# akosiorek/sqair

Hardware: AMD Instinct MI355X
Metric: frames/sec (forward IWAE ELBO, 10-step 50x50 moving glyphs, K=5) (higher is better)
Workload: dtype f32; 1 GPU; cfg2: T=10 HxW=50x50 B=32/GPU K=5 N=4 cells VanillaRNN/GRU/GRU forward (elbo_iwae), HIP-graph replay=True; global_batch=32, seq_len=10, parallelism=dp1, graph_nodes=879

## Files before the change

### include/sqair_hip.h

```cpp
#ifndef SQAIR_HIP_H
#define SQAIR_HIP_H

#include <stddef.h>
#include <stdint.h>

#ifdef __cplusplus
extern "C" {
#endif

#define SQAIR_ABI_VERSION 2

typedef struct SqairConfig {
  int32_t img_h, img_w;
  int32_t glimpse_size;
  int32_t n_steps_per_image;
  int32_t n_what;
  int32_t n_hidden;
  int32_t k_particles;
  int32_t prop_prior_type;
  int32_t disc_prior_type;
  int32_t masked_glimpse;
  int32_t rec_where_prior;
  float prop_prior_step_bias;
  float step_success_prob;
// ... 543 lines not shown
} SqairWhereParamGradsTest;
int sqair_where_param_grads_test(SqairHandle* h, const SqairWhereParamGradsTest* t, void* stream);

typedef struct SqairGruGatesBwdTest {
  int32_t rows, accumulate_dh;
  const float* d_hn; int32_t dhn_ld;
  const float* z; int32_t z_ld;
  const float* r; int32_t r_ld;
  const float* hc; int32_t hc_ld;
  const float* hprev; int32_t h_ld;
  const float* d_rh; int32_t drh_ld;
  float* dpre1; int32_t dp_ld;
  float* d_h; int32_t dh_ld;
  float* dup_z; int32_t dupz_ld, dup_h_off;
  float* dup_r; int32_t dupr_ld;
} SqairGruGatesBwdTest;
int sqair_gru_gates_bwd_test(SqairHandle* h, const SqairGruGatesBwdTest* t, void* stream);

typedef struct SqairSlotCropTest {
  int32_t mode, slot, B, specialised;
  const float* img;
  const float* rec_prev; float* rec_new;
  const float* wb; int32_t wb_ld;
  const float* tp; int32_t tp_ld;
  const float* t2; int32_t t2_ld;
  const float* w3;
  const float* noise;
  const float* flat;
  const float* mask; int32_t mask_row_mul, mask_row_add;
  float* out; int32_t out_row_mul, out_row_add;
  float* tp_out; int32_t tp_out_ld;
} SqairSlotCropTest;
int sqair_slot_crop_test(SqairHandle* h, const SqairSlotCropTest* t, void* stream);

typedef struct SqairSlotTailTest {
  int32_t is_disc, slot, B, what_done;
  const float* hraw; int32_t h_ld;
  const float* enc; int32_t enc_ld;
  const float* rec_prev; float* rec_new;
  const float* noise;
  const float* s1p; int32_t s1p_ld;
  float* s1h_out; int32_t s1h_ld;
  const float* flat; const float* packed;
  const float* hid; int32_t hid_ld;
  const float* add; int32_t add_ld;
  float* out; int32_t out_ld;
} SqairSlotTailTest;
int sqair_slot_tail_test(SqairHandle* h, const SqairSlotTailTest* t, void* stream);

typedef struct SqairLinearWhatTest {
  int32_t mode, slot, B;
  const float* x; int32_t x_ld;
  const float* noise;
  const float* enc; int32_t enc_ld;
  const float* rec_prev; float* rec_new;
  const float* packed;
} SqairLinearWhatTest;
int sqair_linear_what_test(SqairHandle* h, const SqairLinearWhatTest* t, void* stream);

typedef struct SqairLogprobTest {
  int32_t B, T, t, t_global;
  const int32_t* t_row;
  const float* rec_p; const float* rec_d; const float* rec_prev;
  const float* pstats; int32_t ps_ld;
  const float* spre;
  const float* flat;
  float* qz; float* pz; float* disc_lp;
  const SqairOutputs* out;
} SqairLogprobTest;
int sqair_logprob_test(SqairHandle* h, const SqairLogprobTest* t, void* stream);

typedef struct SqairLogprobBwdTest {
  int32_t B, T, t_global0, ps_ld;
  const int32_t* t_row;
  const float* rec_p; const float* rec_d; const float* rec_m;
  const float* pstats; const float* spre;
  const float* g_lw; const float* g_dl;
  float* d_rec_p; float* d_rec_d; float* d_rec_m;
  float* d_pstats; float* d_spre;
  const float* flat; float* flat_grad;
} SqairLogprobBwdTest;
int sqair_logprob_bwd_test(SqairHandle* h, const SqairLogprobBwdTest* t, void* stream);

#define SQAIR_DENSE_ROUTES 23
int sqair_debug_dense_routes(int64_t* out, int n);

#ifdef __cplusplus
}
#endif
#endif
```

### sqair_amd/_capi.py

```python
from __future__ import annotations

import ctypes as C
import os

_HERE = os.path.dirname(os.path.abspath(__file__))
LIB_PATH = os.path.join(_HERE, "libsqair_hip.so")

OUTPUT_FIELDS = [
    "what", "what_loc", "what_scale", "where", "where_loc", "where_scale", "presence_prob", "presence",
    "presence_logit", "obj_id", "step_log_prob", "canvas", "glimpse", "disc_what_log_prob",
    "disc_where_log_prob", "disc_what_prior_log_prob", "disc_where_prior_log_prob", "disc_log_prob",
    "disc_prior_log_prob", "disc_prob", "prop_what_log_prob", "prop_where_log_prob",
    "prop_what_prior_log_prob", "prop_where_prior_log_prob", "prop_log_prob", "prop_prior_log_prob",
    "prop_prob", "discrete_log_prob", "num_prop_steps_per_sample", "num_disc_steps_per_sample",
    "num_steps_per_sample", "prop_pres", "disc_pres", "data_ll_per_sample", "kl_per_sample",
    "log_q_z_given_x_per_sample", "log_p_z_per_sample", "log_weights_per_timestep",
    "final_temporal_state", "final_prior_state", "final_last_used_id",
]
N_REFERENCE_OUTPUTS = 38


class SqairConfig(C.Structure):
    _fields_ = [
        ("img_h", C.c_int32), ("img_w", C.c_int32), ("glimpse_size", C.c_int32),
# ... 185 lines not shown


class SqairDenseContract(C.Structure):
    _fields_ = [("nseg", C.c_int32), ("seg", SqairDenseSeg * 4), ("w", C.c_void_p), ("b", C.c_void_p), ("add", C.c_void_p),
                ("add_ld", C.c_int32), ("add_n", C.c_int32), ("add_rdiv", C.c_int32), ("act_a", C.c_int32), ("act_b", C.c_int32),
                ("act_split", C.c_int32), ("scale", C.c_float), ("scale_ptr", C.c_void_p), ("out", C.c_void_p), ("out_ld", C.c_int32),
                ("M", C.c_int32), ("N", C.c_int32), ("scratch", C.c_void_p), ("scratch_bytes", C.c_int64)]


class SqairDxRange(C.Structure):
    _fields_ = [("n0", C.c_int32), ("n1", C.c_int32), ("dst", C.c_void_p), ("dst_ld", C.c_int32), ("dst2", C.c_void_p),
                ("dst2_ld", C.c_int32), ("add", C.c_void_p), ("add_ld", C.c_int32), ("saved", C.c_void_p), ("saved_ld", C.c_int32),
                ("act_a", C.c_int32), ("act_b", C.c_int32), ("act_split", C.c_int32)]


class SqairDxGru(C.Structure):
    _fields_ = [("mode", C.c_int32), ("g0", C.c_void_p), ("g0_ld", C.c_int32), ("g1", C.c_void_p), ("g1_ld", C.c_int32),
                ("hprev", C.c_void_p), ("h_ld", C.c_int32), ("dpre1", C.c_void_p), ("dp_ld", C.c_int32), ("d_h", C.c_void_p),
                ("dh_ld", C.c_int32), ("acc_dh", C.c_int32), ("dup", C.c_void_p), ("dup_ld", C.c_int32), ("dup_h_off", C.c_int32),
                ("nh", C.c_int32)]


class SqairDxTest(C.Structure):
    _fields_ = [("dpre", C.c_void_p), ("ld", C.c_int32), ("width", C.c_int32), ("M", C.c_int32), ("w", C.c_void_p),
                ("Kdim", C.c_int32), ("scale_ptr", C.c_void_p), ("nranges", C.c_int32), ("r", SqairDxRange * 3), ("gru", SqairDxGru),
                ("scratch", C.c_void_p), ("scratch_bytes", C.c_int64)]


def _fields(spec):
    return [(s.split()[1], C.c_void_p if s.split()[0] == "p" else C.c_int32) for s in spec]


class SqairSlotTailBwdTest(C.Structure):
    _fields_ = _fields(["i is_disc", "i slot", "i B", "i enc_pre", "p rec_prev", "p rec_new", "p d_rec_new", "p d_rec_prev", "p s1h",
                        "i s1h_ld", "p hraw", "i h_ld", "p enc", "i enc_ld", "p noise", "p flat", "p d_s1pre", "i ds_ld", "p d_s1pre2",
                        "i ds2_ld", "p d_raw_out", "i dr_ld", "p d_enc", "i de_ld", "p d_hraw", "i dh_ld"])


class SqairCropChainBwdTest(C.Structure):
    _fields_ = _fields(["i mode", "i slot", "i B", "i mask_dact", "p img", "p rec_prev", "p rec_new", "p d_rec_prev", "p d_rec_new", "p wb",
                        "i wb_ld", "p d_wb", "p mask", "i mask_row_mul", "i mask_row_add", "p d_mask", "p g_out", "i g_row_mul",
                        "i g_row_add", "p tp", "i tp_ld", "p d_tp", "i dtp_ld", "p noise", "p flat", "p w3", "p t2", "i t2_ld", "p d_t2",
                        "i dt2_ld"])


class SqairWhereParamGradsTest(C.Structure):
    _fields_ = _fields(["i T", "i B", "p d_tp", "i tp_ld", "p d_rec_p", "p rec_p", "p noise", "p flat_grad"])


class SqairGruGatesBwdTest(C.Structure):
    _fields_ = _fields(["i rows", "i accumulate_dh", "p d_hn", "i dhn_ld", "p z", "i z_ld", "p r", "i r_ld", "p hc", "i hc_ld", "p hprev",
                        "i h_ld", "p d_rh", "i drh_ld", "p dpre1", "i dp_ld", "p d_h", "i dh_ld", "p dup_z", "i dupz_ld", "i dup_h_off",
                        "p dup_r", "i dupr_ld"])


class SqairLogprobTest(C.Structure):
    _fields_ = _fields(["i B", "i T", "i t", "i t_global", "p t_row", "p rec_p", "p rec_d", "p rec_prev", "p pstats", "i ps_ld", "p spre",
                        "p flat", "p qz", "p pz", "p disc_lp", "p out"])


class SqairLogprobBwdTest(C.Structure):
    _fields_ = _fields(["i B", "i T", "i t_global0", "i ps_ld", "p t_row", "p rec_p", "p rec_d", "p rec_m", "p pstats", "p spre", "p g_lw",
                        "p g_dl", "p d_rec_p", "p d_rec_d", "p d_rec_m", "p d_pstats", "p d_spre", "p flat", "p flat_grad"])


class SqairSlotCropTest(C.Structure):
    _fields_ = _fields(["i mode", "i slot", "i B", "i specialised", "p img", "p rec_prev", "p rec_new", "p wb", "i wb_ld", "p tp", "i tp_ld",
                        "p t2", "i t2_ld", "p w3", "p noise", "p flat", "p mask", "i mask_row_mul", "i mask_row_add", "p out",
                        "i out_row_mul", "i out_row_add", "p tp_out", "i tp_out_ld"])


class SqairSlotTailTest(C.Structure):
    _fields_ = _fields(["i is_disc", "i slot", "i B", "i what_done", "p hraw", "i h_ld", "p enc", "i enc_ld", "p rec_prev", "p rec_new",
                        "p noise", "p s1p", "i s1p_ld", "p s1h_out", "i s1h_ld", "p flat", "p packed", "p hid", "i hid_ld", "p add",
                        "i add_ld", "p out", "i out_ld"])


class SqairLinearWhatTest(C.Structure):
    _fields_ = _fields(["i mode", "i slot", "i B", "p x", "i x_ld", "p noise", "p enc", "i enc_ld", "p rec_prev", "p rec_new", "p packed"])


DENSE_ROUTES = ("fwd_splitk", "fwd_t2", "fwd_rows", "fwd_mt", "fwd_lds", "fwd_big_2x2", "fwd_big_3x2", "fwd_big_3x3", "fwd_big_4x2",
                "dx_nch1", "dx_nch2", "dx_nch3", "dx_nch4", "dx_nch5", "dx_nch6", "dx_nch7", "dx_nch8", "dx_nch9", "dx_nch12", "dx_nch18",
                "dx_t2", "dx_gru1", "dx_gru2")


def dense_routes(library=None):
    v = (C.c_int64 * len(DENSE_ROUTES))()
    n = (library or lib()).sqair_debug_dense_routes(v, len(DENSE_ROUTES))
    assert n == len(DENSE_ROUTES), "the library counts {} dense routes, this binding names {}".format(n, len(DENSE_ROUTES))
    return dict(zip(DENSE_ROUTES, (int(x) for x in v)))


_PROTOS = {
    "sqair_abi_version": (C.c_int, []),
    "sqair_build_id": (C.c_char_p, []),
    "sqair_build_flags": (C.c_char_p, []),
    "sqair_create": (C.c_int, [C.POINTER(SqairConfig), C.POINTER(C.c_void_p)]),
    "sqair_destroy": (C.c_int, [C.c_void_p]),
    "sqair_last_error": (C.c_char_p, [C.c_void_p]),
    "sqair_param_count": (C.c_int64, [C.c_void_p]),
    "sqair_param_entries": (C.c_int, [C.c_void_p]),
    "sqair_param_entry": (C.c_int, [C.c_void_p, C.c_int, C.POINTER(C.c_char_p), C.POINTER(C.c_int64),
                                    C.POINTER(C.c_int64)]),
    "sqair_packed_bytes": (C.c_int64, [C.c_void_p]),
    "sqair_workspace_bytes": (C.c_int64, [C.c_void_p, C.c_int, C.c_int]),
    "sqair_noise_width": (C.c_int, [C.c_void_p]),
    "sqair_pack_params": (C.c_int, [C.c_void_p, C.c_void_p, C.c_void_p, C.c_void_p]),
    "sqair_forward": (C.c_int, [C.c_void_p, C.c_void_p, C.c_void_p, C.c_void_p, C.c_void_p, C.c_int, C.c_int,
                                C.c_int, C.POINTER(SqairOutputs), C.c_void_p, C.c_int64, C.c_void_p]),
    "sqair_train_workspace_bytes": (C.c_int64, [C.c_void_p, C.c_int, C.c_int]),
    "sqair_forward_train": (C.c_int, [C.c_void_p, C.c_void_p, C.c_void_p, C.c_void_p, C.c_void_p, C.c_int, C.c_int,
                                      C.c_int, C.POINTER(SqairOutputs), C.c_void_p, C.c_int64, C.c_void_p]),
    "sqair_graph_capture": (C.c_int, [C.c_void_p, C.c_void_p, C.c_void_p, C.c_void_p, C.c_void_p, C.c_int,
                                      C.c_int, C.c_int, C.POINTER(SqairOutputs), C.c_void_p, C.c_int64,
                                      C.c_void_p]),
    "sqair_graph_launch": (C.c_int, [C.c_void_p, C.c_void_p]),
    "sqair_graph_nodes": (C.c_int, [C.c_void_p]),
    "sqair_elbo": (C.c_int, [C.c_void_p, C.c_void_p, C.c_void_p, C.c_int, C.c_int, C.c_void_p, C.c_void_p,
                             C.c_void_p, C.c_void_p, C.c_void_p, C.POINTER(C.c_void_p), C.c_int, C.c_void_p,
                             C.c_void_p]),
    "sqair_st_crop": (C.c_int, [C.c_void_p, C.c_void_p, C.c_void_p, C.c_void_p, C.c_void_p, C.c_int, C.c_void_p]),
    "sqair_st_insert_loglik": (C.c_int, [C.c_void_p] * 8 + [C.c_int, C.c_void_p]),
    "sqair_linear_test": (C.c_int, [C.c_void_p, C.c_void_p, C.c_void_p, C.c_void_p, C.c_void_p, C.c_int, C.c_int,
                                    C.c_int, C.c_int, C.c_void_p, C.c_int64, C.c_void_p]),
    "sqair_gru_test": (C.c_int, [C.c_void_p, C.c_void_p, C.c_void_p, C.c_void_p, C.c_void_p, C.c_int, C.c_int,
                                 C.c_void_p, C.c_int64, C.c_void_p]),
    "sqair_set_workspace_clearing": (C.c_int, [C.c_void_p, C.c_int]),
    "sqair_clear_workspace": (C.c_int, [C.c_void_p, C.c_void_p, C.c_int64, C.c_int, C.c_int, C.c_int, C.c_void_p]),
    "sqair_set_option": (C.c_int, [C.c_void_p, C.c_char_p, C.c_int]),
    "sqair_chain_status": (C.c_int, [C.c_void_p, C.c_void_p, C.c_int, C.c_int, C.c_int, C.c_void_p]),
    "sqair_check_scales": (C.c_int, [C.c_void_p, C.c_void_p, C.c_int, C.c_int, C.c_int, C.c_void_p, C.c_void_p]),
    "sqair_check_finite": (C.c_int, [C.c_void_p, C.c_void_p, C.c_int64, C.c_char_p, C.c_void_p, C.c_void_p]),
    "sqair_timeline_available": (C.c_int, []),
    "sqair_timeline_begin": (C.c_int, [C.c_void_p, C.c_void_p, C.c_int64]),
    "sqair_timeline_count": (C.c_int, [C.c_void_p]),
    "sqair_timeline_end": (C.c_int, [C.c_void_p]),
    "sqair_timeline_record": (C.c_int, [C.c_void_p, C.c_int, C.POINTER(C.c_char_p), C.POINTER(C.c_int64), C.POINTER(C.c_int),
                                        C.POINTER(C.c_int)]),
    "sqair_lstm_test": (C.c_int, [C.c_void_p] * 6 + [C.c_int, C.c_int, C.c_void_p, C.c_int64, C.c_void_p]),
    "sqair_lstm_cell_bwd_test": (C.c_int, [C.c_void_p] * 7 + [C.c_int, C.c_void_p]),
    "sqair_compact_test_layout": (C.c_int, [C.c_void_p, C.POINTER(C.c_int32), C.c_int]),
    "sqair_compact_test": (C.c_int, [C.c_void_p] * 13 + [C.POINTER(SqairOutputs), C.c_int, C.c_int, C.c_void_p]),
    "sqair_compact_bwd_test": (C.c_int, [C.c_void_p] * 11 + [C.c_int, C.c_void_p]),
    "sqair_get_config":(C.c_int, [C.c_void_p, C.POINTER(SqairConfig)]),
    "sqair_st_crop_bwd": (C.c_int, [C.c_void_p] * 7 + [C.c_int, C.c_void_p]),
    "sqair_st_insert_loglik_bwd": (C.c_int, [C.c_void_p] * 11 + [C.c_int64, C.c_int, C.c_void_p]),
    "sqair_elbo_bwd": (C.c_int, [C.c_void_p, C.c_void_p, C.c_void_p, C.c_int, C.c_int, C.c_void_p, C.c_void_p,
                                 C.c_void_p]),
    "sqair_backward_scratch_bytes": (C.c_int64, [C.c_void_p, C.c_int, C.c_int]),
    "sqair_backward_decoder": (C.c_int, [C.c_void_p] * 6 + [C.c_int, C.c_int, C.c_void_p, C.c_int64, C.c_void_p, C.c_int64,
                                         C.c_void_p, C.c_void_p, C.c_void_p]),
    "sqair_backward_bytes": (C.c_int64, [C.c_void_p, C.c_int, C.c_int]),
    "sqair_backward": (C.c_int, [C.c_void_p] * 7 + [C.c_int, C.c_int, C.c_int, C.c_void_p, C.c_int64, C.c_void_p, C.c_int64,
                                 C.c_void_p, C.c_void_p]),
    "sqair_forward_train_carry": (C.c_int, [C.c_void_p] * 5 + [C.c_int, C.c_int, C.POINTER(SqairCarry), C.POINTER(SqairOutputs),
                                                                C.c_void_p, C.c_int64, C.c_void_p]),
    "sqair_backward_carry": (C.c_int, [C.c_void_p] * 7 + [C.c_int, C.c_int, C.POINTER(SqairCarry), C.c_void_p, C.c_int64,
                                                          C.c_void_p, C.c_int64, C.c_void_p, C.c_void_p]),
    "sqair_forward_train_carry_masked": (C.c_int, [C.c_void_p] * 5 + [C.c_int, C.c_int, C.POINTER(SqairCarry), C.c_void_p,
                                                                       C.POINTER(SqairOutputs), C.c_void_p, C.c_int64, C.c_void_p]),
    "sqair_backward_carry_masked": (C.c_int, [C.c_void_p] * 7 + [C.c_int, C.c_int, C.POINTER(SqairCarry), C.c_void_p, C.c_void_p,
                                                                 C.c_int64, C.c_void_p, C.c_int64, C.c_void_p, C.c_void_p]),
    "sqair_set_generation_noise": (C.c_int, [C.c_void_p, C.c_void_p]),
    "sqair_state_bytes": (C.c_int64, [C.c_void_p, C.c_int]),
    "sqair_set_state": (C.c_int, [C.c_void_p, C.c_void_p, C.c_void_p, C.c_void_p, C.c_int64, C.c_int]),
    "sqair_set_smc": (C.c_int, [C.c_void_p, C.POINTER(SqairSmc), C.c_int]),
# ... 152 lines not shown
```

### sqair_amd/csrc/build.py

```python
import hashlib
import os
import re
import subprocess
import sys

HERE = os.path.dirname(os.path.abspath(__file__))
ROOT = os.path.dirname(os.path.dirname(HERE))
SOURCES = ["sqair_api.hip", "sqair_state.hip", "sqair_linear.hip", "sqair_glue.hip", "sqair_bwd.hip", "sqair_train.hip", "sqair_linear_dx.hip", "sqair_chain.hip",
           "sqair_lane.hip", "sqair_lane_api.hip", "sqair_pack.hip", "sqair_dense_test.hip", "sqair_unit_test.hip"]
OUT = os.path.join(os.path.dirname(HERE), "libsqair_hip.so")
OUT_TIMELINE = os.path.join(os.path.dirname(HERE), "libsqair_hip_timeline.so")
OUT_KNOBS = os.path.join(ROOT, "tools", "bin", "libsqair_hip_knobs.so")
OUT_WIDE = os.path.join(os.path.dirname(HERE), "libsqair_hip_wide.so")
VARIANTS = {"product": (OUT, []), "timeline": (OUT_TIMELINE, ["-DSQAIR_TIMELINE"]), "knobs": (OUT_KNOBS, ["-DSQAIR_KNOBS"]),
            "wide": (OUT_WIDE, ["-DSQAIR_WIDE"])}
HIPCC_FLAGS = ["--offload-arch=gfx950", "-O3", "-std=c++17", "-fPIC", "-shared", "-Wno-unused-result",
               "-mllvm", "-amdgpu-kernarg-preload-count=16", "-mllvm", "-amdgpu-mfma-vgpr-form=1"]
_ID_MARK = re.compile(rb"SQAIR_BUILD_ID=([0-9a-f]{16});")


def source_id():
    hsh = hashlib.sha256()
    for f in sorted(f for f in os.listdir(HERE) if f.endswith((".hip", ".h", ".inc"))):
        hsh.update(f.encode())
        hsh.update(open(os.path.join(HERE, f), "rb").read())
    hsh.update(open(os.path.join(ROOT, "include", "sqair_hip.h"), "rb").read())
    hsh.update(" ".join(HIPCC_FLAGS).encode())
    return hsh.hexdigest()[:16]


def binary_id(path):
    try:
        m = _ID_MARK.search(open(path, "rb").read())
    except OSError:
        return None
    return m.group(1).decode() if m else None


def build(force=False, verbose=False, variant="product"):
    out, defs = VARIANTS[variant]
    sid = source_id()
    if not force and binary_id(out) == sid:
        return out
    os.makedirs(os.path.dirname(out), exist_ok=True)
    hipcc = os.environ.get("HIPCC", "/opt/rocm/bin/hipcc")
    common = [f for f in HIPCC_FLAGS if f != "-shared"] + defs + \
        ['-DSQAIR_BUILD_ID="{}"'.format(sid), '-DSQAIR_BUILD_VARIANT="{}"'.format(variant)]
    objdir = os.path.join(HERE, "_obj", variant)
    os.makedirs(objdir, exist_ok=True)
    objs = [os.path.join(objdir, s.replace(".hip", ".o")) for s in SOURCES]
    cmds = [[hipcc] + common + ["-c", os.path.join(HERE, s), "-o", o] for s, o in zip(SOURCES, objs)]
    if verbose:
        print(" ".join(cmds[0][:-3]) + " -c {" + ",".join(SOURCES) + "}")
    procs = [subprocess.Popen(c) for c in cmds]
    rcs = [p.wait() for p in procs]
    if any(rcs):
        raise subprocess.CalledProcessError(max(rcs), cmds[[i for i, r in enumerate(rcs) if r][0]])
    subprocess.check_call([hipcc, "--offload-arch=gfx950", "-shared", "-fPIC", "-o", out] + objs)
    assert binary_id(out) == sid, "the build id did not make it into {}".format(out)
    return out


if __name__ == "__main__":
    which = [v for v in VARIANTS if "--" + v in sys.argv] or ["product"]
    for v in which:
        print(build(force="--force" in sys.argv, verbose=True, variant=v))
```

### sqair_amd/csrc/sqair_common.h

```cpp
#pragma once
#include <hip/hip_runtime.h>
#include <stdint.h>
#include <string>
#include <vector>

#include "../../include/sqair_hip.h"

#define SQ_CHECK_HIP(expr)                                                                   \
  do {                                                                                       \
    hipError_t _e = (expr);                                                                  \
    if (_e != hipSuccess) {                                                                  \
      sq_set_error(h, std::string(#expr) + ": " + hipGetErrorString(_e));                    \
      return -2;                                                                             \
    }                                                                                        \
  } while (0)

namespace rec {
#ifdef SQAIR_WIDE
constexpr int NWMAX = 128;
constexpr int WHERE = 0;
constexpr int WHAT = 4;
constexpr int PRES = 132;
constexpr int LOGIT = 133;
constexpr int ZW = 134;
// ... 13 lines not shown
constexpr int LOGIT = 55;
constexpr int ZW = 56;
constexpr int ZWP = 64;
constexpr int WHERE_LOC = 56;
constexpr int WHERE_SCALE = 60;
constexpr int WHAT_LOC = 64;
constexpr int WHAT_SCALE = 114;
constexpr int PROB = 164;
constexpr int ID = 165;
constexpr int W = 168;
#endif
#ifdef SQAIR_WIDE
#define SQ_WHAT_LANES(c, lane, nw) for (int c = (lane); c < (nw); c += 64)
#else
#define SQ_WHAT_LANES(c, lane, nw) for (int c = (lane), sq_once_ = 1; sq_once_ != 0 && c < (nw); sq_once_ = 0)
#endif
}

enum Act { ACT_NONE = 0, ACT_ELU = 1, ACT_TANH = 2, ACT_SIGMOID = 3, ACT_SOFTPLUS_MIN = 4 };
enum Epi { EPI_ACT = 0, EPI_GRU1 = 1, EPI_GRU2 = 2 };

struct LinSeg {
  const float* p;
  int ld;
  int width;
  int rdiv;
  unsigned rmul;
};

struct LinArgs {
  LinSeg seg[4];
  int nseg;
  const float* wp;
  const float* bias;
  const float* wzero;
  const float* add;
  int add_ld, add_rdiv, add_n;
  unsigned add_rmul;
  float* out;
  int out_ld;
  int M, N;
  int epi;
  int act_a, act_b, act_split;
  const float* scale_ptr;
  float scale;
  const float* e0; int e0_ld;
  const float* e1; int e1_ld;
  float* o1; int o1_ld;
  float* o2; int o2_ld;
  float* o3; int o3_ld;
  int nh;
};

struct PackedLayer {
  int64_t w_off;
  int64_t b_off;
  int kc;
  int nt;
  int N;
  std::vector<int> seg_width;
};

#define SQ_LOCAL __attribute__((visibility("hidden")))

struct SqairHandle;
void sq_set_error(SqairHandle* h, const std::string& msg);
int sq_allow_big_lds(const void* kernel, int bytes);

__device__ __forceinline__ void philox4x32_10(unsigned c0, unsigned c1, unsigned c2, unsigned c3, unsigned k0, unsigned k1,
                                              unsigned out[4]) {
#pragma unroll
  for (int r = 0; r < 10; ++r) {
    const unsigned long long p0 = (unsigned long long)0xD2511F53u * c0, p1 = (unsigned long long)0xCD9E8D57u * c2;
    const unsigned n0 = (unsigned)(p1 >> 32) ^ c1 ^ k0, n1 = (unsigned)p1, n2 = (unsigned)(p0 >> 32) ^ c3 ^ k1, n3 = (unsigned)p0;
    c0 = n0; c1 = n1; c2 = n2; c3 = n3;
    k0 += 0x9E3779B9u; k1 += 0xBB67AE85u;
  }
  out[0] = c0; out[1] = c1; out[2] = c2; out[3] = c3;
}

enum DenseRoute {
  DR_SPLITK = 0, DR_T2, DR_ROWS, DR_MT, DR_LDS, DR_BIG22, DR_BIG32, DR_BIG33, DR_BIG42,
  DR_DX_NCH1, DR_DX_NCH2, DR_DX_NCH3, DR_DX_NCH4, DR_DX_NCH5, DR_DX_NCH6, DR_DX_NCH7, DR_DX_NCH8, DR_DX_NCH9, DR_DX_NCH12, DR_DX_NCH18,
  DR_DX_T2, DR_DX_GRU1, DR_DX_GRU2, DR_COUNT
};
void sq_dense_route_hit(int route);
long long sq_dense_route_hits(int route);

int sq_launch_linear(const LinArgs& a, const PackedLayer& L, hipStream_t s);
bool sq_linear_leaves_split_k(int M, const PackedLayer& L);
int sq_launch_pack(const float* flat, float* packed_w, const int* idx, int64_t n, hipStream_t s);
int sq_launch_pack_bias(const float* flat, float* packed_b, const int* idxa, const int* idxb, int64_t n,
                        hipStream_t s);

#ifdef SQAIR_TIMELINE
struct SqTl { unsigned long long* slot; unsigned gx, gy, nw, pad; };
SqTl sq_tl_next(const char* kernel, dim3 grid, dim3 block);
#define SQ_TLP , const SqTl sq_tl
#define SQ_TL_SCOPE SqTlScope sq_tl_scope(sq_tl)
#define SQ_LAUNCH(kern, grid, block, lds, s, ...) \
  hipLaunchKernelGGL(kern, grid, block, lds, s, __VA_ARGS__, sq_tl_next(#kern, grid, block))
#ifdef __HIPCC__
struct SqTlScope {
  const SqTl tl;
  const unsigned long long t0;
  static __device__ __forceinline__ unsigned long long clock() {
    unsigned long long t;
    asm volatile("s_memrealtime %0\n\ts_waitcnt lgkmcnt(0)" : "=s"(t));
    return t;
  }
  __device__ __forceinline__ explicit SqTlScope(const SqTl tl_) : tl(tl_), t0(__builtin_amdgcn_s_memrealtime()) {}
  __device__ __forceinline__ ~SqTlScope() {
    const uintptr_t b = (uintptr_t)tl.slot;
    if (b == 0) return;
    const unsigned tid = threadIdx.x;
    if ((tid & 63u) != 0u) return;
    const unsigned wg = blockIdx.x + tl.gx * (blockIdx.y + tl.gy * blockIdx.z);
    typedef unsigned long long u64x2 __attribute__((ext_vector_type(2)));
    typedef __attribute__((address_space(1))) u64x2 gvec;
    gvec* p = (gvec*)b + ((size_t)wg * tl.nw + (tid >> 6));
    u64x2 v;
    v.x = t0;
    v.y = clock();
    *p = v;
  }
};
#endif
#else
#define SQ_TLP
#define SQ_TL_SCOPE
#ifdef SQAIR_KNOBS
#include <cstdio>
#include <cstdlib>
#define SQ_LAUNCH(kern, grid, block, lds, s, ...)                                              \
  do {                                                                                         \
    static const bool sq_sync_ = getenv("SQAIR_SYNC_LAUNCHES") != nullptr;                     \
    if (sq_sync_) { fprintf(stderr, "launch %s\n", #kern); fflush(stderr); }                   \
    hipLaunchKernelGGL(kern, grid, block, lds, s, __VA_ARGS__);                                \
    if (sq_sync_) (void)hipStreamSynchronize(s);                                               \
  } while (0)
#else
#define SQ_LAUNCH(kern, grid, block, lds, s, ...) hipLaunchKernelGGL(kern, grid, block, lds, s, __VA_ARGS__)
#endif
#endif

#ifdef SQAIR_KNOBS
#define SQ_KNOB_INT(name, dflt) (getenv(name) ? atoi(getenv(name)) : (dflt))
#define SQ_KNOB_SET(name) (getenv(name) != nullptr)
#define SQ_KNOB_STR(name) getenv(name)
#else
#define SQ_KNOB_INT(name, dflt) (dflt)
#define SQ_KNOB_SET(name) false
#define SQ_KNOB_STR(name) ((const char*)nullptr)
#endif

#ifdef __HIPCC__
__device__ __forceinline__ float sq_exp(float x) {
  const float x0 = x;
  x = __builtin_amdgcn_fmed3f(x, -104.0f, 88.72283f);
  const float t = x * 1.44269504088896340736f;
  const float r = fmaf(x, 1.44269504088896340736f, -t) + x * 1.92596299112661746e-8f;
  const float e = __builtin_amdgcn_exp2f(t);
  return x0 != x0 ? x0 : fmaf(e, r * 0.69314718055994530942f, e);
}
__device__ __forceinline__ float sq_log(float x) { return __builtin_amdgcn_logf(x) * 0.69314718055994530942f; }
__device__ __forceinline__ float sq_sigmoid(float x) { return __builtin_amdgcn_rcpf(1.0f + sq_exp(-x)); }
__device__ __forceinline__ float sq_sigmoid_geo(float x) { return 1.0f / (1.0f + expf(-x)); }
__device__ __forceinline__ float sq_to_coord(float l, int q) { return (q & 2) ? tanhf(l) : fmaxf(sq_sigmoid_geo(l), 1e-4f); }
__device__ __forceinline__ float sq_tanh(float x) {
// ... 88 lines not shown
```

### sqair_amd/csrc/sqair_linear.hip

```cpp
#include <type_traits>
#include "sqair_common.h"
#include "sqair_lin_device.h"
#include <atomic>
#include <stdio.h>
#include <stdlib.h>

typedef float f32x4 __attribute__((ext_vector_type(4)));

__global__ void k_pack(const float* __restrict__ flat, float* __restrict__ packed, const int* __restrict__ idx,
                       int64_t n SQ_TLP) {
  SQ_TL_SCOPE;
  constexpr int U = 8;
  int64_t i = (int64_t)blockIdx.x * blockDim.x + threadIdx.x;
  const int64_t stride = (int64_t)gridDim.x * blockDim.x;
  for (; i < n; i += stride * U) {
    int j[U];
    float v[U];
#pragma unroll
    for (int u = 0; u < U; ++u) j[u] = idx[min(i + u * stride, n - 1)];
#pragma unroll
    for (int u = 0; u < U; ++u) v[u] = flat[max(j[u], 0)];
#pragma unroll
    for (int u = 0; u < U; ++u)
      if (i + u * stride < n) packed[i + u * stride] = j[u] >= 0 ? v[u] : 0.0f;
// ... 719 lines not shown
}
template <int NCH>
static void launch_nch(const LinArgs& a, const PackedLayer& L, hipStream_t s) {
  switch (a.nseg) {
    case 1: launch_seg<NCH, 1>(a, L, s); break;
    case 2: launch_seg<NCH, 2>(a, L, s); break;
    case 3: launch_seg<NCH, 3>(a, L, s); break;
    default: launch_seg<NCH, 4>(a, L, s); break;
  }
}

static std::atomic<long long> g_dense_route[DR_COUNT];
void sq_dense_route_hit(int route) { ++g_dense_route[route]; }
long long sq_dense_route_hits(int route) { return route >= 0 && route < DR_COUNT ? g_dense_route[route].load() : -1; }

static unsigned rmul_of(int rdiv) { return rdiv <= 1 ? 0u : (unsigned)((1ull << 32) / (unsigned)rdiv) + 1u; }

#ifndef SQAIR_MT_ROWS_DEFAULT
#define SQAIR_MT_ROWS_DEFAULT 6000
#endif
bool sq_linear_leaves_split_k(int M, const PackedLayer& L) {
  static const int mt_rows = SQ_KNOB_INT("SQAIR_MT_ROWS", SQAIR_MT_ROWS_DEFAULT);
  const bool mid_wide = L.kc > 4 && M >= 1792 && L.nt >= 48;
  return M >= mt_rows || mid_wide;
}

int sq_launch_linear(const LinArgs& a_in, const PackedLayer& L, hipStream_t s) {
  LinArgs a = a_in;
  for (int i = 0; i < a.nseg; ++i) a.seg[i].rmul = rmul_of(a.seg[i].rdiv);
  a.add_rmul = rmul_of(a.add_rdiv);
  const int mt = (a.M + 15) / 16;
  const int grid = mt * L.nt;
  if (grid <= 0) return 0;
  for (int i = 0; i < a.nseg; ++i) {
    const LinSeg& sg = a.seg[i];
    if ((reinterpret_cast<uintptr_t>(sg.p) & 15) != 0 || (sg.ld & 3) != 0 || sg.width < 1 || sg.rdiv < 1) return -5;
  }
  if (sq_linear_leaves_split_k(a.M, L)) {
    if (L.kc <= 4) {
      const dim3 grid_r(L.nt, (mt + 3) / 4);
      sq_dense_route_hit(DR_ROWS);
      SQ_LAUNCH(k_linear_rows<4>, grid_r, dim3(256), 0, s, a, L.kc, L.nt);
      return 0;
    }
    static const int big = SQ_KNOB_INT("SQAIR_BIG", 2);
    if (big > 0 && L.nt >= 4) {
#ifdef SQAIR_KNOBS
      if (const char* e = SQ_KNOB_STR("SQAIR_BIG_SHAPE")) {
        const int tm = e[0] - '0', tn = e[2] - '0';
#define SQ_BIG_CASE(A, B) if (tm == A && tn == B) { launch_big<A, B>(a, L, s); return 0; }
        SQ_BIG_CASE(1, 2) SQ_BIG_CASE(1, 3) SQ_BIG_CASE(1, 4)
        SQ_BIG_CASE(2, 2) SQ_BIG_CASE(2, 3) SQ_BIG_CASE(2, 4) SQ_BIG_CASE(3, 2) SQ_BIG_CASE(3, 3) SQ_BIG_CASE(3, 4)
        SQ_BIG_CASE(4, 2) SQ_BIG_CASE(4, 3) SQ_BIG_CASE(4, 4)
#undef SQ_BIG_CASE
      }
#endif
      switch (pick_big_shape(a.M, L.nt, L.kc, a.act_a != ACT_NONE)) {
        case 22: sq_dense_route_hit(DR_BIG22); launch_big<2, 2>(a, L, s); break;
        case 32: sq_dense_route_hit(DR_BIG32); launch_big<3, 2>(a, L, s); break;
        case 33: sq_dense_route_hit(DR_BIG33); launch_big<3, 3>(a, L, s); break;
        default: sq_dense_route_hit(DR_BIG42); launch_big<4, 2>(a, L, s); break;
      }
      return 0;
    }
    static const int lds_wgs = SQ_KNOB_INT("SQAIR_LDS_WGS", 512);
    if (((a.M + 127) / 128) * ((L.nt + 3) / 4) >= lds_wgs) {
      sq_dense_route_hit(DR_LDS);
      SQ_LAUNCH((k_linear_lds<2>), dim3((L.nt + 3) / 4, (a.M + 127) / 128), dim3(256), 0, s, a, L.kc, L.nt);
      return 0;
    }
    const MtShape sh = pick_mt_shape(a.M, L.nt, L.kc);
    sq_dense_route_hit(DR_MT);
    if (sh.nt >= 2) launch_mt<4, 1, 2>(a, L, mt, sh.coal != 0, s);
    else launch_mt<4, 1, 1>(a, L, mt, sh.coal != 0, s);
    return 0;
  }
  const int per_wave = (L.kc + 3) / 4;
  static const int t2_rows = SQ_KNOB_INT("SQAIR_T2_ROWS", 512), t2_kc = SQ_KNOB_INT("SQAIR_T2_KC", 40);
  if (a.M >= t2_rows && L.nt >= 4 && L.kc >= t2_kc) {
    sq_dense_route_hit(DR_T2);
    launch_t2_any(a, L, s);
    return 0;
  }
  sq_dense_route_hit(DR_SPLITK);
  switch (per_wave) {
    case 1: launch_nch<1>(a, L, s); break;
    case 2: launch_nch<2>(a, L, s); break;
    case 3: launch_nch<3>(a, L, s); break;
    case 4: launch_nch<4>(a, L, s); break;
    case 5: launch_nch<5>(a, L, s); break;
    case 6: launch_nch<6>(a, L, s); break;
    case 7: launch_nch<7>(a, L, s); break;
    case 8: launch_nch<8>(a, L, s); break;
    case 9: launch_nch<9>(a, L, s); break;
    default: launch_nch<10>(a, L, s); break;
  }
  return 0;
}
```

Measured before the change: 101,500 frames/s.

## Add LDS-staged strip linear kernel for mid-size M, shallow-K dense layers

Measured after the change: 102,600 frames/s, median of 6. 1.01x the previous value.

```diff
diff --git a/include/sqair_hip.h b/include/sqair_hip.h
--- a/include/sqair_hip.h
+++ b/include/sqair_hip.h
@@ -649,7 +649,7 @@
 } SqairLogprobBwdTest;
 int sqair_logprob_bwd_test(SqairHandle* h, const SqairLogprobBwdTest* t, void* stream);
 
-#define SQAIR_DENSE_ROUTES 23
+#define SQAIR_DENSE_ROUTES 24
 int sqair_debug_dense_routes(int64_t* out, int n);
 
 #ifdef __cplusplus
diff --git a/sqair_amd/_capi.py b/sqair_amd/_capi.py
--- a/sqair_amd/_capi.py
+++ b/sqair_amd/_capi.py
@@ -291,7 +291,7 @@
 
 DENSE_ROUTES = ("fwd_splitk", "fwd_t2", "fwd_rows", "fwd_mt", "fwd_lds", "fwd_big_2x2", "fwd_big_3x2", "fwd_big_3x3", "fwd_big_4x2",
                 "dx_nch1", "dx_nch2", "dx_nch3", "dx_nch4", "dx_nch5", "dx_nch6", "dx_nch7", "dx_nch8", "dx_nch9", "dx_nch12", "dx_nch18",
-                "dx_t2", "dx_gru1", "dx_gru2")
+                "dx_t2", "dx_gru1", "dx_gru2", "fwd_strip")
 
 
 def dense_routes(library=None):
diff --git a/sqair_amd/csrc/build.py b/sqair_amd/csrc/build.py
--- a/sqair_amd/csrc/build.py
+++ b/sqair_amd/csrc/build.py
@@ -7,7 +7,8 @@
 HERE = os.path.dirname(os.path.abspath(__file__))
 ROOT = os.path.dirname(os.path.dirname(HERE))
 SOURCES = ["sqair_api.hip", "sqair_state.hip", "sqair_linear.hip", "sqair_glue.hip", "sqair_bwd.hip", "sqair_train.hip", "sqair_linear_dx.hip", "sqair_chain.hip",
-           "sqair_lane.hip", "sqair_lane_api.hip", "sqair_pack.hip", "sqair_dense_test.hip", "sqair_unit_test.hip"]
+           "sqair_lane.hip", "sqair_lane_api.hip", "sqair_pack.hip", "sqair_dense_test.hip", "sqair_unit_test.hip",
+           "sqair_linear_strip.hip"]
 OUT = os.path.join(os.path.dirname(HERE), "libsqair_hip.so")
 OUT_TIMELINE = os.path.join(os.path.dirname(HERE), "libsqair_hip_timeline.so")
 OUT_KNOBS = os.path.join(ROOT, "tools", "bin", "libsqair_hip_knobs.so")
diff --git a/sqair_amd/csrc/sqair_common.h b/sqair_amd/csrc/sqair_common.h
--- a/sqair_amd/csrc/sqair_common.h
+++ b/sqair_amd/csrc/sqair_common.h
@@ -119,9 +119,10 @@
 enum DenseRoute {
   DR_SPLITK = 0, DR_T2, DR_ROWS, DR_MT, DR_LDS, DR_BIG22, DR_BIG32, DR_BIG33, DR_BIG42,
   DR_DX_NCH1, DR_DX_NCH2, DR_DX_NCH3, DR_DX_NCH4, DR_DX_NCH5, DR_DX_NCH6, DR_DX_NCH7, DR_DX_NCH8, DR_DX_NCH9, DR_DX_NCH12, DR_DX_NCH18,
-  DR_DX_T2, DR_DX_GRU1, DR_DX_GRU2, DR_COUNT
+  DR_DX_T2, DR_DX_GRU1, DR_DX_GRU2, DR_STRIP, DR_COUNT
 };
 void sq_dense_route_hit(int route);
+SQ_LOCAL int sq_launch_linear_strip(const LinArgs& a, const PackedLayer& L, hipStream_t s, bool* taken);
 long long sq_dense_route_hits(int route);
 
 int sq_launch_linear(const LinArgs& a, const PackedLayer& L, hipStream_t s);
diff --git a/sqair_amd/csrc/sqair_linear.hip b/sqair_amd/csrc/sqair_linear.hip
--- a/sqair_amd/csrc/sqair_linear.hip
+++ b/sqair_amd/csrc/sqair_linear.hip
@@ -825,6 +825,14 @@
     launch_t2_any(a, L, s);
     return 0;
   }
+  {
+    bool taken = false;
+    const int rc = sq_launch_linear_strip(a, L, s, &taken);
+    if (taken) {
+      if (rc == 0) sq_dense_route_hit(DR_STRIP);
+      return rc;
+    }
+  }
   sq_dense_route_hit(DR_SPLITK);
   switch (per_wave) {
     case 1: launch_nch<1>(a, L, s); break;
diff --git a/sqair_amd/csrc/sqair_linear_strip.hip b/sqair_amd/csrc/sqair_linear_strip.hip
--- /dev/null
+++ b/sqair_amd/csrc/sqair_linear_strip.hip
@@ -0,0 +1,210 @@
+#include "sqair_common.h"
+#include "sqair_lin_device.h"
+
+typedef float f32x4 __attribute__((ext_vector_type(4)));
+
+#define SQ_STRIP_KC_MAX 39
+#define SQ_STRIP_ROWS_MIN 512
+#define SQ_STRIP_ROWS_END 768
+#define SQ_STRIP_GRID_MIN 192
+
+template <int RT, int S, int G>
+__global__ __launch_bounds__(256 * G) void k_linear_strip(const LinArgs a, const int kc_total, const int n_tiles SQ_TLP) {
+  SQ_TL_SCOPE;
+  static_assert(RT == 1 || RT == 2, "row tiles per workgroup");
+  constexpr int NT = RT * S;
+  constexpr int NR = (16 * RT + 4 * G - 1) / (4 * G);
+  constexpr int NJ = (SQ_STRIP_KC_MAX * 4 + 63) / 64;
+  extern __shared__ __attribute__((aligned(16))) float lds[];
+  const int lane = threadIdx.x & 63, kq = lane >> 4, l15 = lane & 15;
+  const int wave_all = __builtin_amdgcn_readfirstlane(threadIdx.x >> 6);
+  const int group = wave_all >> 2, wave = wave_all & 3;
+  const int tid = threadIdx.x & 255;
+  const int tile_n0 = (blockIdx.x * G + group) * S, tile_m0 = blockIdx.y * RT;
+  const int nmine = (kc_total - wave + 3) >> 2;
+  const int pitch = kc_total * 16 + 4;
+
+  const f32x4* wq[S];
+#pragma unroll
+  for (int t = 0; t < S; ++t) wq[t] = reinterpret_cast<const f32x4*>(a.wp) + ((size_t)min(tile_n0 + t, n_tiles - 1) * kc_total) * 64 + lane;
+  f32x4 bP[S], bQ[S], bR[S];
+  const f32x4* __restrict__ wz = reinterpret_cast<const f32x4*>(a.wzero) + lane;
+#define SQ_ST_ISSUE(BV, I)                                                                        \
+  {                                                                                               \
+    const bool valid = (I) < nmine;                                                               \
+    const size_t go = (size_t)(wave + 4 * (I)) * 64;                                              \
+    _Pragma("unroll") for (int t = 0; t < S; ++t) BV[t] = *(valid ? wq[t] + go : wz);             \
+  }
+  SQ_ST_ISSUE(bP, 0)
+  SQ_ST_ISSUE(bQ, 1)
+  __builtin_amdgcn_sched_barrier(0);
+
+  {
+    const float* sp0 = a.seg[0].p; const float* sp1 = a.seg[1].p; const float* sp2 = a.seg[2].p; const float* sp3 = a.seg[3].p;
+    const int sl0 = a.seg[0].ld, sl1 = a.seg[1].ld, sl2 = a.seg[2].ld, sl3 = a.seg[3].ld;
+    const unsigned sm0 = a.seg[0].rmul, sm1 = a.seg[1].rmul, sm2 = a.seg[2].rmul, sm3 = a.seg[3].rmul;
+    const int w0 = a.seg[0].width, w1 = a.seg[1].width, w2 = a.seg[2].width, w3 = a.seg[3].width;
+    const int c1 = (w0 + 15) >> 4;
+    const int c2 = c1 + (a.nseg > 1 ? (w1 + 15) >> 4 : 0);
+    const int c3 = c2 + (a.nseg > 2 ? (w2 + 15) >> 4 : 0);
+    const int cum1 = a.nseg > 1 ? c1 : 0x7fffffff, cum2 = a.nseg > 2 ? c2 : 0x7fffffff, cum3 = a.nseg > 3 ? c3 : 0x7fffffff;
+    const int lim0 = ((w0 + 3) & ~3) - 4, lim1 = ((w1 + 3) & ~3) - 4, lim2 = ((w2 + 3) & ~3) - 4, lim3 = ((w3 + 3) & ~3) - 4;
+    const int kc4 = kc_total * 4;
+    int arow[NR];
+#pragma unroll
+    for (int r = 0; r < NR; ++r) arow[r] = min(tile_m0 * 16 + min(wave_all + 4 * G * r, 16 * RT - 1), a.M - 1);
+    f32x4 st[NJ][NR];
+#pragma unroll
+    for (int j = 0; j < NJ; ++j) {
+      if (64 * j < kc4) {
+        const int qc = min(lane + 64 * j, kc4 - 1);
+        const int g = qc >> 2;
+        const bool s1 = g >= cum1, s2 = g >= cum2, s3 = g >= cum3;
+        const float* sp = s3 ? sp3 : (s2 ? sp2 : (s1 ? sp1 : sp0));
+        const int sl = s3 ? sl3 : (s2 ? sl2 : (s1 ? sl1 : sl0));
+        const unsigned sm = s3 ? sm3 : (s2 ? sm2 : (s1 ? sm1 : sm0));
+        const int cb = s3 ? cum3 : (s2 ? cum2 : (s1 ? cum1 : 0));
+        const int lim = s3 ? lim3 : (s2 ? lim2 : (s1 ? lim1 : lim0));
+        const int kk = min((g - cb) * 16 + (qc & 3) * 4, lim);
+#pragma unroll
+        for (int r = 0; r < NR; ++r) {
+          const int rr = sm ? (int)__umulhi((unsigned)arow[r], sm) : arow[r];
+          st[j][r] = *reinterpret_cast<const f32x4*>(sp + (size_t)rr * sl + kk);
+        }
+      }
+    }
+    __builtin_amdgcn_sched_barrier(0);
+#pragma unroll
+    for (int j = 0; j < NJ; ++j) {
+      if (64 * j < kc4) {
+        const int q = lane + 64 * j;
+        if (q < kc4) {
+#pragma unroll
+          for (int r = 0; r < NR; ++r)
+            if ((16 * RT) % (4 * G) == 0 || wave_all + 4 * G * r < 16 * RT)
+              *reinterpret_cast<f32x4*>(&lds[(wave_all + 4 * G * r) * pitch + q * 4]) = st[j][r];
+        }
+      }
+    }
+  }
+  __builtin_amdgcn_sched_barrier(0);
+  __builtin_amdgcn_s_waitcnt(0xC07F);
+  __builtin_amdgcn_s_barrier();
+  __builtin_amdgcn_sched_barrier(0);
+
+  const int er = tid >> 4, ec = tid & 15;
+  const bool has_add = a.add != nullptr;
+  float p_bias[NT], p_add[NT];
+#define SQ_ST_NC(q) min(min(tile_n0 + (q) % S, n_tiles - 1) * 16 + ec, a.N - 1)
+#define SQ_ST_MC(q) min((tile_m0 + (q) / S) * 16 + er, a.M - 1)
+#pragma unroll
+  for (int q = 0; q < NT; ++q) { p_bias[q] = a.bias[SQ_ST_NC(q)]; p_add[q] = 0.0f; }
+  if (has_add) {
+#pragma unroll
+    for (int q = 0; q < NT; ++q) {
+      const int nc = SQ_ST_NC(q), mc = SQ_ST_MC(q);
+      const int mcd = a.add_rmul ? (int)__umulhi((unsigned)mc, a.add_rmul) : mc;
+      p_add[q] = *(nc < a.add_n ? a.add + (size_t)mcd * a.add_ld + nc : a.wzero + ec);
+    }
+  }
+  float p_scale = *(a.scale_ptr != nullptr ? a.scale_ptr : a.bias);
+  __builtin_amdgcn_sched_barrier(0);
+
+  f32x4 acc0[RT][S], acc1[RT][S];
+#pragma unroll
+  for (int r = 0; r < RT; ++r)
+#pragma unroll
+    for (int t = 0; t < S; ++t) { acc0[r][t] = f32x4{0.0f, 0.0f, 0.0f, 0.0f}; acc1[r][t] = acc0[r][t]; }
+  const float* afrag = lds + l15 * pitch + kq * 4;
+#define SQ_ST_SWEEP(BV, ACC, C)                                                                   \
+  _Pragma("unroll") for (int r = 0; r < RT; ++r) {                                                \
+    _Pragma("unroll") for (int t = 0; t < S; ++t)                                                 \
+      ACC[r][t] = __builtin_amdgcn_mfma_f32_16x16x4f32(af[r].C, BV[t].C, ACC[r][t], 0, 0, 0);     \
+  }
+#define SQ_ST_CONSUME(BV, I)                                                                      \
+  {                                                                                               \
+    f32x4 af[RT];                                                                                 \
+    _Pragma("unroll") for (int r = 0; r < RT; ++r)                                                \
+      af[r] = *reinterpret_cast<const f32x4*>(afrag + r * 16 * pitch + min(wave + 4 * (I), kc_total - 1) * 16); \
+    SQ_ST_SWEEP(BV, acc0, x) SQ_ST_SWEEP(BV, acc1, y) SQ_ST_SWEEP(BV, acc0, z) SQ_ST_SWEEP(BV, acc1, w) \
+  }
+#pragma unroll 1
+  for (int i = 0; i < nmine; i += 3) {
+    SQ_ST_ISSUE(bR, i + 2)
+    __builtin_amdgcn_sched_barrier(0);
+    SQ_ST_CONSUME(bP, i)
+    __builtin_amdgcn_sched_barrier(0);
+    SQ_ST_ISSUE(bP, i + 3)
+    __builtin_amdgcn_sched_barrier(0);
+    SQ_ST_CONSUME(bQ, i + 1)
+    __builtin_amdgcn_sched_barrier(0);
+    SQ_ST_ISSUE(bQ, i + 4)
+    __builtin_amdgcn_sched_barrier(0);
+    SQ_ST_CONSUME(bR, i + 2)
+    __builtin_amdgcn_sched_barrier(0);
+  }
+#undef SQ_ST_ISSUE
+#undef SQ_ST_SWEEP
+#undef SQ_ST_CONSUME
+
+  if (has_add) {
+#pragma unroll
+    for (int q = 0; q < NT; ++q) p_add[q] = SQ_ST_NC(q) < a.add_n ? p_add[q] : 0.0f;
+  }
+#undef SQ_ST_NC
+#undef SQ_ST_MC
+  p_scale = a.scale_ptr != nullptr ? p_scale : 1.0f;
+
+  __syncthreads();
+  float* const red = lds + group * (4 * NT * 256);
+  {
+    float* r = red + wave * (NT * 256) + (4 * kq) * 16 + l15;
+#pragma unroll
+    for (int rt = 0; rt < RT; ++rt) {
+#pragma unroll
+      for (int t = 0; t < S; ++t) {
+        const int q = rt * S + t;
+        r[q * 256 + 0] = acc0[rt][t].x + acc1[rt][t].x;
+        r[q * 256 + 16] = acc0[rt][t].y + acc1[rt][t].y;
+        r[q * 256 + 32] = acc0[rt][t].z + acc1[rt][t].z;
+        r[q * 256 + 48] = acc0[rt][t].w + acc1[rt][t].w;
+      }
+    }
+  }
+  __syncthreads();
+#pragma unroll
+  for (int q = 0; q < NT; ++q) {
+    float* e = red + q * 256 + tid;
+    const float v = e[0] + e[NT * 256] + e[2 * NT * 256] + e[3 * NT * 256] + p_bias[q] + p_add[q];
+    e[0] = v;
+  }
+#pragma unroll 1
+  for (int q = 0; q < NT; ++q) {
+    const int rt = q / S, t = q - rt * S;
+    const int n0 = (tile_n0 + t) * 16;
+    const int m = (tile_m0 + rt) * 16 + er, n = n0 + ec;
+    if (tile_n0 + t < n_tiles && m < a.M && n < a.N) {
+      const float* e = red + q * 256 + tid;
+      if (a.act_split <= n0) { LinArgs u = a; u.act_a = a.act_b; x_epilogue(u, m, n, e[0], 0.0f, 0.0f, p_scale); }
+      else if (a.act_split >= n0 + 16) { LinArgs u = a; u.act_b = a.act_a; x_epilogue(u, m, n, e[0], 0.0f, 0.0f, p_scale); }
+      else x_epilogue(a, m, n, e[0], 0.0f, 0.0f, p_scale);
+    }
+  }
+}
+
+int sq_launch_linear_strip(const LinArgs& a, const PackedLayer& L, hipStream_t s, bool* taken) {
+  constexpr int RT = 2, S = 2, G = 3;
+  const int mt = (a.M + 15) / 16;
+  const dim3 g((L.nt + G * S - 1) / (G * S), (mt + RT - 1) / RT);
+  const int grid = (int)(g.x * g.y);
+  *taken = a.epi == EPI_ACT && a.M >= SQ_STRIP_ROWS_MIN && a.M < SQ_STRIP_ROWS_END && L.kc <= SQ_STRIP_KC_MAX &&
+           grid >= SQ_STRIP_GRID_MIN && grid <= 256;
+  if (!*taken) return 0;
+  const int image = 16 * RT * (16 * L.kc + 4) * 4, red = G * 4 * RT * S * 256 * 4;
+  const int lds = image > red ? image : red;
+  constexpr int LDS_CEILING = 16 * RT * (16 * SQ_STRIP_KC_MAX + 4) * 4;
+  static_assert(LDS_CEILING <= 150 * 1024 && LDS_CEILING >= G * 4 * RT * S * 256 * 4, "the deepest image fits the CU's LDS and covers the reduction buffer");
+  if (lds > 64 * 1024 && sq_allow_big_lds((const void*)k_linear_strip<RT, S, G>, LDS_CEILING) != 0) return -2;
+  SQ_LAUNCH((k_linear_strip<RT, S, G>), g, dim3(256 * G), lds, s, a, L.kc, L.nt);
+  return 0;
+}
```
